# mfkiwl/HiSpMV

Hardware: AMD Instinct MI355X
Metric: SpMV GFLOP/s, SuiteSparse set (20 matrices), fp32 y=alpha*A*x+beta*y, flops=2*(nnz+rows) (higher is better)
Workload: dtype f32

## Files before the change

hispmv_amd/csrc/hispmv_kernels.hip:

```cpp
#include <hip/hip_runtime.h>

#include "hispmv_format.h"
#include "hispmv_kernels.h"
#include <algorithm>
#include <cstdlib>
#include <mutex>
#include <type_traits>
#include <vector>

#ifndef HISPMV_TTS_EXPERIMENT
#define HISPMV_TTS_EXPERIMENT 0
#endif

namespace hispmv {

#ifdef HISPMV_WG_TRACE
__device__ unsigned long long* g_wgt_buf = nullptr;
__device__ unsigned g_wgt_cap = 0;
struct WgTrace {
    unsigned long long t0;
    __device__ __forceinline__ void begin() { t0 = __builtin_amdgcn_s_memrealtime(); }
    __device__ __forceinline__ void end(int kind, int entry, long long item) {
        __syncthreads();
        if (threadIdx.x == 0 && g_wgt_buf) {
            const unsigned long long t1 = __builtin_amdgcn_s_memrealtime();
            unsigned hw, xcc;
            asm volatile("s_getreg_b32 %0, hwreg(HW_REG_HW_ID)" : "=s"(hw));
            asm volatile("s_getreg_b32 %0, hwreg(HW_REG_XCC_ID)" : "=s"(xcc));
            const unsigned long long i = __hip_atomic_fetch_add(g_wgt_buf, 1ull, __ATOMIC_RELAXED, __HIP_MEMORY_SCOPE_AGENT);
            if (i < g_wgt_cap) {
                unsigned long long* r = g_wgt_buf + 4 + 4 * i;
                r[0] = t0; r[1] = t1;
                r[2] = ((unsigned long long)xcc << 32) | hw;
                r[3] = ((unsigned long long)kind << 56) | ((unsigned long long)(entry & 0xffff) << 40) | (unsigned long long)(item & 0xffffffffffll);
            }
        }
    }
};
#define WGT_BEGIN() WgTrace wgt; wgt.begin()
#define WGT_END(kind, entry, item) wgt.end(kind, entry, item)
#else
#define WGT_BEGIN()
#define WGT_END(kind, entry, item)
#endif

__device__ __forceinline__ int f2i(float f) { return __builtin_bit_cast(int, f); }
__device__ __forceinline__ float i2f(int i) { return __builtin_bit_cast(float, i); }

struct ScanFlags { unsigned long long f[7]; };
__device__ __forceinline__ ScanFlags scan_flags(unsigned long long heads) {
    ScanFlags s;
    s.f[0] = heads;
    s.f[1] = s.f[0] | ((s.f[0] << 1) & 0xfffefffefffefffeull);
    s.f[2] = s.f[1] | ((s.f[1] << 2) & 0xfffcfffcfffcfffcull);
    s.f[3] = s.f[2] | ((s.f[2] << 4) & 0xfff0fff0fff0fff0ull);
    s.f[4] = s.f[3] | ((s.f[3] << 8) & 0xff00ff00ff00ff00ull);
    s.f[5] = s.f[4] | (((s.f[4] >> 15) & 1ull) ? 0x00000000ffff0000ull : 0ull)
                    | (((s.f[4] >> 47) & 1ull) ? 0xffff000000000000ull : 0ull);
    s.f[6] = s.f[5] | (((s.f[5] >> 31) & 1ull) ? 0xffffffff00000000ull : 0ull);
    return s;
}
template <int CTRL, int ROWMASK>
__device__ __forceinline__ void seg_scan_step(float& v, unsigned long long F) {
    const float vp = i2f(__builtin_amdgcn_update_dpp(0, f2i(v), CTRL, ROWMASK, 0xf, false));
    v = __builtin_amdgcn_inverse_ballot_w64(F) ? v : v + vp;
}
__device__ __forceinline__ void seg_scan_wave(float& v, const ScanFlags& s) {
    seg_scan_step<0x111, 0xf>(v, s.f[0]);
    seg_scan_step<0x112, 0xf>(v, s.f[1]);
    seg_scan_step<0x114, 0xf>(v, s.f[2]);
    seg_scan_step<0x118, 0xf>(v, s.f[3]);
    seg_scan_step<0x142, 0xa>(v, s.f[4]);
    seg_scan_step<0x143, 0xc>(v, s.f[5]);
}

__device__ __forceinline__ float wave_sum(float v) {
    v += i2f(__builtin_amdgcn_update_dpp(0, f2i(v), 0x111, 0xf, 0xf, false));
    v += i2f(__builtin_amdgcn_update_dpp(0, f2i(v), 0x112, 0xf, 0xf, false));
    v += i2f(__builtin_amdgcn_update_dpp(0, f2i(v), 0x114, 0xf, 0xf, false));
    v += i2f(__builtin_amdgcn_update_dpp(0, f2i(v), 0x118, 0xf, 0xf, false));
    v += i2f(__builtin_amdgcn_update_dpp(0, f2i(v), 0x142, 0xa, 0xf, false));
    v += i2f(__builtin_amdgcn_update_dpp(0, f2i(v), 0x143, 0xc, 0xf, false));
    return i2f(__builtin_amdgcn_readlane(f2i(v), 63));
}

constexpr int kTtsChunkSlots = 1024;
constexpr int kLookbackSpinMax = 1 << 22;

__device__ __forceinline__ int lanes_below(unsigned long long mask) {
    return __builtin_amdgcn_mbcnt_hi((unsigned)(mask >> 32), __builtin_amdgcn_mbcnt_lo((unsigned)mask, 0));
}

typedef __attribute__((address_space(3))) unsigned long long lds_u64;
__device__ __forceinline__ void mbox_store(lds_u64* p, unsigned long long v) {
    __hip_atomic_store(p, v, __ATOMIC_RELAXED, __HIP_MEMORY_SCOPE_WORKGROUP);
}
__device__ __forceinline__ unsigned long long mbox_load(lds_u64* p) {
    return __hip_atomic_load(p, __ATOMIC_RELAXED, __HIP_MEMORY_SCOPE_WORKGROUP);
}

__device__ __forceinline__ float lookback_chain(const LookbackArgs& lb, lds_u64* local,
                                                long long first, long long cur, int chain_len, int lane) {
    float part = 0.0f;
    for (int k = lane; k < chain_len; k += 64) {
        const long long src = cur - chain_len + k;
        unsigned long long v;
        int spins = 0;
        if (src >= first) {
            v = mbox_load(local + (src - first));
            while ((unsigned)(v >> 32) != lb.epoch && spins < kLookbackSpinMax) {
                __builtin_amdgcn_s_sleep(1);
                v = mbox_load(local + (src - first));
                ++spins;
            }
        } else {
            const unsigned long long* g = lb.gran + src;
            v = __hip_atomic_load(g, __ATOMIC_RELAXED, __HIP_MEMORY_SCOPE_AGENT);
            while ((unsigned)(v >> 32) != lb.epoch && spins < kLookbackSpinMax) {
                __builtin_amdgcn_s_sleep(2);
                v = __hip_atomic_load(g, __ATOMIC_RELAXED, __HIP_MEMORY_SCOPE_AGENT);
                ++spins;
            }
        }
        if ((unsigned)(v >> 32) != lb.epoch) *lb.err = 1;
        part += i2f((int)(unsigned)v);
    }
    return wave_sum(part);
}

#define HISPMV_GLOBAL __attribute__((address_space(1)))
__device__ __forceinline__ uint4 load_words(const uint4* p) {
    typedef unsigned int u4v __attribute__((ext_vector_type(4)));
    const u4v v = __builtin_nontemporal_load((const HISPMV_GLOBAL u4v*)p);
    return uint4{v.x, v.y, v.z, v.w};
}
__device__ __forceinline__ uint2 load_words2(const uint2* p) {
    typedef unsigned int u2v __attribute__((ext_vector_type(2)));
    const u2v v = __builtin_nontemporal_load((const HISPMV_GLOBAL u2v*)p);
    return uint2{v.x, v.y};
}
__device__ __forceinline__ int4 load_int4(const int4* p) {
    typedef int i4v __attribute__((ext_vector_type(4)));
    const i4v v = *(const HISPMV_GLOBAL i4v*)p;
    return int4{v.x, v.y, v.z, v.w};
}
__device__ __forceinline__ float4 load_float4(const float4* p) {
    typedef float f4v __attribute__((ext_vector_type(4)));
    const f4v v = *(const HISPMV_GLOBAL f4v*)p;
    return float4{v.x, v.y, v.z, v.w};
}
__device__ __forceinline__ void store_float(float* p, float v) { *(HISPMV_GLOBAL float*)p = v; }
__device__ __forceinline__ int2 load_int2(const int2* p) {
    typedef int i2v __attribute__((ext_vector_type(2)));
    const i2v v = *(const HISPMV_GLOBAL i2v*)p;
    return int2{v.x, v.y};
}

template <bool COMPACT, bool HALF = false> struct SliceRaw;
template <> struct SliceRaw<true>  { uint4 v[kSliceSteps]; uint2 m[kSliceSteps]; };
template <> struct SliceRaw<false> { uint4 v[kSliceSteps]; uint4 m[kSliceSteps]; };
template <> struct SliceRaw<true, true> { uint4 q[kSliceSteps]; };
template <bool COMPACT, bool HALF = false>
__device__ __forceinline__ void request_slice(SliceRaw<COMPACT, HALF>& s, const char* base, int lane) {
    if constexpr (HALF) {
        const uint4* pq = (const uint4*)base + lane;
#pragma unroll
        for (int j = 0; j < kSliceSteps; ++j) s.q[j] = load_words(pq + j * 64);
    } else {
    const uint4* pv = (const uint4*)base + lane;
#pragma unroll
    for (int j = 0; j < kSliceSteps; ++j) s.v[j] = load_words(pv + j * 64);
    if constexpr (COMPACT) {
        const uint2* pm = (const uint2*)(base + kSliceElems * 4) + lane;
#pragma unroll
        for (int j = 0; j < kSliceSteps; ++j) s.m[j] = load_words2(pm + j * 64);
    } else {
        const uint4* pm = (const uint4*)(base + kSliceElems * 4) + lane;
#pragma unroll
        for (int j = 0; j < kSliceSteps; ++j) s.m[j] = load_words(pm + j * 64);
    }
    }
}
template <bool COMPACT, bool HALF>
__device__ __forceinline__ void slice_values(const SliceRaw<COMPACT, HALF>& s, int j, float (&v)[kLaneElems]) {
    if constexpr (HALF) {
        v[0] = i2f((int)(s.q[j].x << 16)); v[1] = i2f((int)(s.q[j].x & 0xffff0000u));
        v[2] = i2f((int)(s.q[j].y << 16)); v[3] = i2f((int)(s.q[j].y & 0xffff0000u));
    } else {
        v[0] = i2f((int)s.v[j].x); v[1] = i2f((int)s.v[j].y); v[2] = i2f((int)s.v[j].z); v[3] = i2f((int)s.v[j].w);
    }
}
template <bool COMPACT, bool HALF = false>
__device__ __forceinline__ void decode_metas(const SliceRaw<COMPACT, HALF>& s, unsigned (&c)[kSliceSteps * kLaneElems]) {
    if constexpr (COMPACT) {
#pragma unroll
        for (int j = 0; j < kSliceSteps; ++j) {
            unsigned a, b;
            if constexpr (HALF) { a = s.q[j].z; b = s.q[j].w; } else { a = s.m[j].x; b = s.m[j].y; }
            c[4 * j + 0] = ((a & 0x8000u) << 16) | (a & 0x7fffu);
            c[4 * j + 1] = (a & 0x80000000u) | ((a >> 16) & 0x7fffu);
            c[4 * j + 2] = ((b & 0x8000u) << 16) | (b & 0x7fffu);
            c[4 * j + 3] = (b & 0x80000000u) | ((b >> 16) & 0x7fffu);
        }
    } else {
#pragma unroll
        for (int j = 0; j < kSliceSteps; ++j) { c[4 * j + 0] = s.m[j].x; c[4 * j + 1] = s.m[j].y; c[4 * j + 2] = s.m[j].z; c[4 * j + 3] = s.m[j].w; }
    }
}

__device__ __forceinline__ void scan_step(const float (&p)[kLaneElems], bool e0, bool e1, bool e2, bool e3, float& carry_step,
                                          float (&t)[kLaneElems]) {
    const float s0 = p[0];
    const float s1 = e0 ? p[1] : s0 + p[1];
    const float s2 = e1 ? p[2] : s1 + p[2];
    const float s3 = e2 ? p[3] : s2 + p[3];
    float v = e3 ? 0.0f : s3;
    const ScanFlags F = scan_flags(__builtin_amdgcn_ballot_w64(e0 | e1 | e2 | e3));
    seg_scan_wave(v, F);
    v = __builtin_amdgcn_inverse_ballot_w64(F.f[6]) ? v : v + carry_step;
    const float cin = i2f(__builtin_amdgcn_update_dpp(f2i(carry_step), f2i(v), 0x138, 0xf, 0xf, false));
    carry_step = i2f(__builtin_amdgcn_readlane(f2i(v), 63));
    t[0] = cin + s0;
    t[1] = e0 ? s1 : cin + s1;
    t[2] = (e0 | e1) ? s2 : cin + s2;
    t[3] = (e0 | e1 | e2) ? s3 : cin + s3;
}

__device__ __forceinline__ void stage_fragments(const int4* __restrict__ frags, int first, int count, const float* x, float* win,
                                                int cols, int lane, int wave, int n_waves) {
    constexpr int kU = 8;
    int4 fr = wave < count ? load_int4(frags + first + wave) : int4{0, 0, 0, 0};
    for (int f = wave; f < count; f += n_waves) {
        const int col0 = __builtin_amdgcn_readfirstlane(fr.x), n4 = __builtin_amdgcn_readfirstlane(fr.y) >> 2;
        const int off = __builtin_amdgcn_readfirstlane(fr.z);
        if (f + n_waves < count) fr = load_int4(frags + first + f + n_waves);
        const float4* src = (const float4*)(x + col0);
        float4* dst = (float4*)(win + off);
        const int inside = cols - col0 >= 4 * n4 ? n4 : (cols > col0 ? (cols - col0) >> 2 : 0);
        int i0 = 0;
        for (; inside - i0 > 128; i0 += 64 * kU) {
            float4 v[kU];
#pragma unroll
            for (int u = 0; u < kU; ++u) {
                const int i = i0 + 64 * u + lane;
                v[u] = load_float4(src + (i < inside ? i : inside - 1));
            }
#pragma unroll
            for (int u = 0; u < kU; ++u) {
                const int i = i0 + 64 * u + lane;
                if (i < inside) dst[i] = v[u];
            }
        }
        if (inside - i0 > 64) {
            const int ia = i0 + lane, ib = i0 + 64 + lane;
            const float4 va = load_float4(src + ia), vb = load_float4(src + (ib < inside ? ib : inside - 1));
            dst[ia] = va;
            if (ib < inside) dst[ib] = vb;
        } else if (inside - i0 > 0) {
            const int ia = i0 + lane;
            if (ia < inside) dst[ia] = load_float4(src + ia);
        }
        if (inside + lane < n4) {
            const int i = inside + lane, c0 = col0 + 4 * i;
            const HISPMV_GLOBAL float* xg = (const HISPMV_GLOBAL float*)x;
            const float a0 = c0 + 0 < cols ? xg[c0 + 0] : 0.f;
            const float a1 = c0 + 1 < cols ? xg[c0 + 1] : 0.f;
            const float a2 = c0 + 2 < cols ? xg[c0 + 2] : 0.f;
            dst[i] = float4{a0, a1, a2, 0.f};
        }
    }
}

struct SubBlock {
    int wave, n_waves, lds_off;
    int lane;
    static __device__ __forceinline__ SubBlock whole() { return SubBlock{(int)(threadIdx.x >> 6), (int)(blockDim.x >> 6), 0, (int)(threadIdx.x & 63)}; }
};

template <bool HAS_BETA, bool USE_LDS, bool LOOKBACK, bool COMPACT, bool STRAYS = false, bool HALF = false>
__device__ __forceinline__ void slices_group(
    const char* __restrict__ stream, const int4* __restrict__ hdr, const int4* __restrict__ groups,
    const int4* __restrict__ frags,
    const float* __restrict__ x, const float* bias, float* y,
    float* __restrict__ carry, float alpha, float beta, long long n_slices, int group_slices,
    int lds_floats, int ytile_floats, int cols, int rows, const LookbackArgs& lb, long long group, int4 g, const SubBlock sb) {
    extern __shared__ float xs_base[];
    float* const xs = xs_base + sb.lds_off;
    const __amdgpu_buffer_rsrc_t rx = __builtin_amdgcn_make_buffer_rsrc((void*)x, 0, cols * 4, 0x00020000);
    const __amdgpu_buffer_rsrc_t rb = __builtin_amdgcn_make_buffer_rsrc((void*)bias, 0, rows * 4, 0x00020000);
    const __amdgpu_buffer_rsrc_t ry = __builtin_amdgcn_make_buffer_rsrc((void*)y, 0, rows * 4, 0x00020000);
    const __amdgpu_buffer_rsrc_t rc = __builtin_amdgcn_make_buffer_rsrc((void*)carry, 0, LOOKBACK ? 0 : (int)(n_slices * 4), 0x00020000);
    constexpr unsigned kNoAccess = 0xffffffffu;
    constexpr int kE = kSliceSteps * kLaneElems;
    const int lane = sb.lane;
    const int wave = sb.wave, n_waves = sb.n_waves;
    float* const ytile = xs + (USE_LDS ? lds_floats : 0) + wave * ytile_floats;
    lds_u64* const mbox = (lds_u64*)(xs + (USE_LDS ? lds_floats : 0) + n_waves * ytile_floats);
    const long long first = group * group_slices;
    const long long last = (first + group_slices < n_slices) ? first + group_slices : n_slices;
    constexpr int slice_bytes = HALF ? kHalfSliceBytes : COMPACT ? kCompactSliceBytes : kWideSliceBytes;
    const char* const gbase = stream + (USE_LDS ? (size_t)(unsigned)__builtin_amdgcn_readfirstlane(g.z) * kSliceUnit
                                                : (size_t)first * kWideSliceBytes);

    const int n_here = (int)(last > first ? last - first : 0);
    const int rot = (LOOKBACK || n_here == 0) ? 0 : (int)((unsigned long long)group * 29ull % (unsigned)n_here);
    int k_slice = wave;
    int local = k_slice < n_here ? (k_slice + rot >= n_here ? k_slice + rot - n_here : k_slice + rot) : n_here;
    SliceRaw<COMPACT, HALF> w;
    int4 h = int4{0, 0, 0, 0};
    const bool strays = STRAYS && COMPACT && (__builtin_amdgcn_readfirstlane(g.w) & 2) != 0;
    const __amdgpu_buffer_rsrc_t rs = __builtin_amdgcn_make_buffer_rsrc((void*)(hdr + n_slices), 0, strays ? (int)(n_slices * (kStraySlots * 4)) : 0, 0x00020000);
    float* const stray_area = xs + (lds_floats - n_waves * kStraySlots) + wave * kStraySlots;
    unsigned sc_next = 0xffffffffu;
    float sx_cur = 0.0f;
    if (strays) {
        const unsigned sc0 = local < n_here ? __builtin_amdgcn_raw_buffer_load_b32(rs, (unsigned)((first + local) * kStraySlots + lane) << 2, 0, 0) : 0xffffffffu;
        const int k2 = k_slice + n_waves;
        const int l2 = k2 < n_here ? (k2 + rot >= n_here ? k2 + rot - n_here : k2 + rot) : -1;
        sc_next = l2 >= 0 ? __builtin_amdgcn_raw_buffer_load_b32(rs, (unsigned)((first + l2) * kStraySlots + lane) << 2, 0, 0) : 0xffffffffu;
        sx_cur = i2f((int)__builtin_amdgcn_raw_buffer_load_b32(rx, sc0 << 2, 0, 0));
    }
    if (local < n_here) {
        h = load_int4(hdr + first + local);
        request_slice<COMPACT, HALF>(w, gbase + (size_t)local * slice_bytes, lane);
    }

    if (LOOKBACK) {
        for (int i = threadIdx.x; i < group_slices; i += blockDim.x) mbox_store(mbox + i, 0ull);
        if (!USE_LDS) __syncthreads();
    }
    bool in_lds = false;
    if (USE_LDS) {
        in_lds = g.y > 0;
        stage_fragments(frags, g.x, g.y, x, xs, cols, lane, wave, n_waves);
        __syncthreads();
    }

    long long def_slice = -1, pend_slice = -1;
    int def_row = 0, def_len = 0, pend_row = 0, pend_len = 0;
    float def_t = 0.0f, def_b = 0.0f, pend_t = 0.0f, pend_b = 0.0f;
    float out_t0 = 0.0f, out_t1 = 0.0f, out_b0 = 0.0f, out_b1 = 0.0f, out_carry = 0.0f;
    unsigned out_d0 = kNoAccess, out_d1 = kNoAccess, out_dc = kNoAccess;

    while (local < n_here) {
        asm volatile("" :: "v"(h.x), "v"(h.y), "v"(h.z), "v"(h.w));
        int row = __builtin_amdgcn_readfirstlane(h.x);
        const int row_first = row;
        const int chain_len = __builtin_amdgcn_readfirstlane(h.y);
        const int n_rows = __builtin_amdgcn_readfirstlane(h.z);
        const bool spills = USE_LDS && __builtin_amdgcn_readfirstlane(h.w) != 0;
        unsigned c[kE];
        decode_metas<COMPACT, HALF>(w, c);
        if (!LOOKBACK) {
            asm volatile("" : "+v"(c[0]), "+v"(c[kE - 1]) :: "memory");
            __builtin_amdgcn_raw_buffer_store_b32((unsigned)f2i(HAS_BETA ? alpha * out_t0 + beta * out_b0 : alpha * out_t0), ry, out_d0, 0, 0);
            __builtin_amdgcn_raw_buffer_store_b32((unsigned)f2i(HAS_BETA ? alpha * out_t1 + beta * out_b1 : alpha * out_t1), ry, out_d1, 0, 0);
            __builtin_amdgcn_raw_buffer_store_b32((unsigned)f2i(out_carry), rc, out_dc, 0, 0);
        }
        float sx_next = 0.0f;
        if (strays) {
            stray_area[lane] = sx_cur;
            sx_next = i2f((int)__builtin_amdgcn_raw_buffer_load_b32(rx, sc_next << 2, 0, 0));
        }
        float bpre0 = 0.0f, bpre1 = 0.0f;
        if (HAS_BETA) {
            bpre0 = i2f((int)__builtin_amdgcn_raw_buffer_load_b32(rb, lane < n_rows ? (unsigned)(row_first + lane) << 2 : kNoAccess, 0, 0));
            bpre1 = i2f((int)__builtin_amdgcn_raw_buffer_load_b32(rb, lane + 64 < n_rows ? (unsigned)(row_first + lane + 64) << 2 : kNoAccess, 0, 0));
        }
        int r0[kSliceSteps];
        bool ends[kE];
        unsigned step_has_end = 0;
#pragma unroll
        for (int j = 0; j < kSliceSteps; ++j) {
            int below = 0, total = 0;
#pragma unroll
            for (int k = 0; k < kLaneElems; ++k) {
                ends[4 * j + k] = (c[4 * j + k] & kRowEndBit) != 0;
                const unsigned long long m = __builtin_amdgcn_ballot_w64(ends[4 * j + k]);
                below += lanes_below(m);
                total += __builtin_popcountll(m);
            }
            r0[j] = row + below;
            row += total;
            step_has_end |= (total != 0 ? 1u : 0u) << j;
        }

        float xv[kE];
        if (COMPACT || (USE_LDS && in_lds && !spills)) {
#pragma unroll
            for (int i = 0; i < kE; ++i) xv[i] = xs[c[i] & ~kRowEndBit];
        } else if (USE_LDS && in_lds) {
#pragma unroll
            for (int i = 0; i < kE; ++i) {
                const unsigned ci = c[i] & ~kRowEndBit;
                xv[i] = i2f((int)__builtin_amdgcn_raw_buffer_load_b32(rx, (ci & kGlobalColBit) ? ci << 2 : kNoAccess, 0, 0));
            }
#pragma unroll
            for (int i = 0; i < kE; ++i) {
                const unsigned ci = c[i] & ~kRowEndBit;
                const float l = xs[(ci & kGlobalColBit) ? 0u : ci];
                xv[i] = (ci & kGlobalColBit) ? xv[i] : l;
            }
        } else {
#pragma unroll
            for (int i = 0; i < kE; ++i) xv[i] = i2f((int)__builtin_amdgcn_raw_buffer_load_b32(rx, (c[i] & ~kRowEndBit) << 2, 0, 0));
        }
        float p[kE];
#pragma unroll
        for (int j = 0; j < kSliceSteps; ++j) {
            if constexpr (HALF) {
                float vj[kLaneElems];
                slice_values(w, j, vj);
                p[4 * j + 0] = vj[0] * xv[4 * j + 0]; p[4 * j + 1] = vj[1] * xv[4 * j + 1];
                p[4 * j + 2] = vj[2] * xv[4 * j + 2]; p[4 * j + 3] = vj[3] * xv[4 * j + 3];
            } else {
            p[4 * j + 0] = i2f((int)w.v[j].x) * xv[4 * j + 0];
            p[4 * j + 1] = i2f((int)w.v[j].y) * xv[4 * j + 1];
            p[4 * j + 2] = i2f((int)w.v[j].z) * xv[4 * j + 2];
            p[4 * j + 3] = i2f((int)w.v[j].w) * xv[4 * j + 3];
            }
        }
        if (!LOOKBACK) {
#pragma unroll
            for (int i = 0; i < kE; ++i) asm volatile("" : "+v"(p[i]));
            asm volatile("" ::: "memory");
        }
        const long long cur = first + local;
        k_slice += n_waves;
        local = k_slice < n_here ? (k_slice + rot >= n_here ? k_slice + rot - n_here : k_slice + rot) : n_here;
        if (strays) {
            const int k2 = k_slice + n_waves;
            const int l2 = k2 < n_here ? (k2 + rot >= n_here ? k2 + rot - n_here : k2 + rot) : -1;
            sx_cur = sx_next;
            sc_next = l2 >= 0 ? __builtin_amdgcn_raw_buffer_load_b32(rs, (unsigned)((first + l2) * kStraySlots + lane) << 2, 0, 0) : 0xffffffffu;
        }
        if (local < n_here) {
            h = load_int4(hdr + first + local);
            request_slice<COMPACT, HALF>(w, gbase + (size_t)local * slice_bytes, lane);
        }

        float carry_step = 0.0f;
#pragma unroll
        for (int j = 0; j < kSliceSteps; ++j) {
            if (step_has_end & (1u << j)) {
                const float pj[kLaneElems] = {p[4 * j], p[4 * j + 1], p[4 * j + 2], p[4 * j + 3]};
                float tj[kLaneElems];
                scan_step(pj, ends[4 * j], ends[4 * j + 1], ends[4 * j + 2], ends[4 * j + 3], carry_step, tj);
                int pos = r0[j] - row_first;
#pragma unroll
                for (int k = 0; k < kLaneElems; ++k) {
                    if (ends[4 * j + k]) ytile[pos] = tj[k];
                    pos += ends[4 * j + k] ? 1 : 0;
                }
            } else {
                carry_step = wave_sum(((p[4 * j] + p[4 * j + 1]) + p[4 * j + 2]) + p[4 * j + 3]) + carry_step;
            }
        }

        bool deferred = false, rolling = false;
        if (LOOKBACK) {
            if (lane == 0) {
                const unsigned long long granule = ((unsigned long long)lb.epoch << 32) | (unsigned)f2i(carry_step);
                mbox_store(mbox + (cur - first), granule);
                __hip_atomic_store(lb.gran + cur, granule, __ATOMIC_RELAXED, __HIP_MEMORY_SCOPE_AGENT);
            }
            if (pend_slice >= 0) {
                const float chain = lookback_chain(lb, mbox, first, pend_slice, pend_len, lane);
                if (lane == 0) {
                    const float tt = pend_t + chain;
                    __builtin_amdgcn_raw_buffer_store_b32((unsigned)f2i(HAS_BETA ? alpha * tt + beta * pend_b : alpha * tt), ry,
                                                          (unsigned)pend_row << 2, 0, 0);
                }
                pend_slice = -1;
            }
            deferred = chain_len > (int)(cur - first);
            rolling = chain_len > 0 && !deferred;
            if (deferred) { def_slice = cur; def_row = row_first; def_len = chain_len; }
            if (rolling) { pend_slice = cur; pend_row = row_first; pend_len = chain_len; }
        }

        const bool held = LOOKBACK && (deferred || rolling);
        if (!LOOKBACK) {
            out_t0 = lane < n_rows ? ytile[lane] : 0.0f;
            out_t1 = lane + 64 < n_rows ? ytile[lane + 64] : 0.0f;
            out_b0 = bpre0; out_b1 = bpre1;
            out_d0 = lane < n_rows ? (unsigned)(row_first + lane) << 2 : kNoAccess;
            out_d1 = lane + 64 < n_rows ? (unsigned)(row_first + lane + 64) << 2 : kNoAccess;
            out_carry = carry_step;
            out_dc = lane == 0 ? (unsigned)cur << 2 : kNoAccess;
        }
        for (int i0 = 128; !LOOKBACK && i0 < n_rows; i0 += 256) {
            float bb[4] = {0.0f, 0.0f, 0.0f, 0.0f};
            if (HAS_BETA) {
#pragma unroll
                for (int u = 0; u < 4; ++u) {
                    const int i = i0 + 64 * u + lane;
                    bb[u] = i2f((int)__builtin_amdgcn_raw_buffer_load_b32(rb, i < n_rows ? (unsigned)(row_first + i) << 2 : kNoAccess, 0, 0));
                }
            }
#pragma unroll
            for (int u = 0; u < 4; ++u) {
                const int i = i0 + 64 * u + lane;
                const float tt = i < n_rows ? ytile[i] : 0.0f;
                __builtin_amdgcn_raw_buffer_store_b32((unsigned)f2i(HAS_BETA ? alpha * tt + beta * bb[u] : alpha * tt), ry,
                                                      i < n_rows ? (unsigned)(row_first + i) << 2 : kNoAccess, 0, 0);
            }
        }
        for (int i = lane; LOOKBACK && i < n_rows; i += 64) {
            const float tt = ytile[i];
            const unsigned dst = (held && i == 0) ? kNoAccess : (unsigned)(row_first + i) << 2;
            if (HAS_BETA) {
                const float b = (i < 64) ? bpre0 : (i < 128) ? bpre1
                              : i2f((int)__builtin_amdgcn_raw_buffer_load_b32(rb, (unsigned)(row_first + i) << 2, 0, 0));
                if (LOOKBACK && deferred && i == 0) { def_t = tt; def_b = b; }
                if (LOOKBACK && rolling && i == 0) { pend_t = tt; pend_b = b; }
                __builtin_amdgcn_raw_buffer_store_b32((unsigned)f2i(alpha * tt + beta * b), ry, dst, 0, 0);
            } else {
                if (LOOKBACK && deferred && i == 0) def_t = tt;
                if (LOOKBACK && rolling && i == 0) pend_t = tt;
                __builtin_amdgcn_raw_buffer_store_b32((unsigned)f2i(alpha * tt), ry, dst, 0, 0);
            }
        }
    }
    if (!LOOKBACK) {
        __builtin_amdgcn_raw_buffer_store_b32((unsigned)f2i(HAS_BETA ? alpha * out_t0 + beta * out_b0 : alpha * out_t0), ry, out_d0, 0, 0);
        __builtin_amdgcn_raw_buffer_store_b32((unsigned)f2i(HAS_BETA ? alpha * out_t1 + beta * out_b1 : alpha * out_t1), ry, out_d1, 0, 0);
        __builtin_amdgcn_raw_buffer_store_b32((unsigned)f2i(out_carry), rc, out_dc, 0, 0);
    }
    if (LOOKBACK && pend_slice >= 0) {
        const float chain = lookback_chain(lb, mbox, first, pend_slice, pend_len, lane);
        if (lane == 0) {
            const float tt = pend_t + chain;
            __builtin_amdgcn_raw_buffer_store_b32((unsigned)f2i(HAS_BETA ? alpha * tt + beta * pend_b : alpha * tt), ry,
                                                  (unsigned)pend_row << 2, 0, 0);
        }
    }
    if (LOOKBACK && def_slice >= 0) {
        const float chain = lookback_chain(lb, mbox, first, def_slice, def_len, lane);
        if (lane == 0) {
            const float tt = def_t + chain;
            __builtin_amdgcn_raw_buffer_store_b32((unsigned)f2i(HAS_BETA ? alpha * tt + beta * def_b : alpha * tt), ry,
                                                  (unsigned)def_row << 2, 0, 0);
        }
    }
}

template <bool HAS_BETA, bool USE_LDS, bool LOOKBACK, bool STRAYS = false, int HALF = 0>
__device__ __forceinline__ void slices_body(
    const char* __restrict__ stream, const int4* __restrict__ hdr, const int4* __restrict__ groups,
    const int4* __restrict__ frags, const float* __restrict__ x, const float* bias, float* y,
    float* __restrict__ carry, float alpha, float beta, long long n_slices, int group_slices,
    int lds_floats, int ytile_floats, int cols, int rows, const LookbackArgs& lb, long long group, const SubBlock sb) {
    __shared__ long long s_group;
    if (LOOKBACK) {
        if (lb.use_ticket) {
            if (threadIdx.x == 0)
                s_group = (long long)(__hip_atomic_fetch_add(lb.ticket, 1ull, __ATOMIC_RELAXED, __HIP_MEMORY_SCOPE_AGENT) - lb.ticket_base);
            __syncthreads();
            group = s_group;
        }
    }
    if constexpr (USE_LDS) {
        const int4 g = group * group_slices < n_slices ? load_int4(groups + group) : int4{0, 0, 0, 0};
        if constexpr (HALF != 0) {
            if ((__builtin_amdgcn_readfirstlane(g.w) & kGroupHalf) != 0) {
                slices_group<HAS_BETA, true, LOOKBACK, true, STRAYS, true>(stream, hdr, groups, frags, x, bias, y, carry, alpha, beta, n_slices, group_slices,
                                                                           lds_floats, ytile_floats, cols, rows, lb, group, g, sb);
                return;
            }
        }
        if constexpr (HALF == 2) {
            slices_group<HAS_BETA, true, LOOKBACK, false>(stream, hdr, groups, frags, x, bias, y, carry, alpha, beta, n_slices, group_slices,
                                                          lds_floats, ytile_floats, cols, rows, lb, group, g, sb);
            return;
        }
        if (__builtin_amdgcn_readfirstlane(g.w) != 0)
            slices_group<HAS_BETA, true, LOOKBACK, true, STRAYS>(stream, hdr, groups, frags, x, bias, y, carry, alpha, beta, n_slices, group_slices,
                                                         lds_floats, ytile_floats, cols, rows, lb, group, g, sb);
        else
            slices_group<HAS_BETA, true, LOOKBACK, false>(stream, hdr, groups, frags, x, bias, y, carry, alpha, beta, n_slices, group_slices,
                                                          lds_floats, ytile_floats, cols, rows, lb, group, g, sb);
    } else {
        slices_group<HAS_BETA, false, LOOKBACK, false>(stream, hdr, groups, frags, x, bias, y, carry, alpha, beta, n_slices, group_slices,
                                                       lds_floats, ytile_floats, cols, rows, lb, group, int4{0, 0, 0, 0}, sb);
    }
}
template <bool HAS_BETA, bool USE_LDS, bool LOOKBACK, bool STRAYS = false, int HALF = 0>
__device__ __forceinline__ void slices_body(
    const char* __restrict__ stream, const int4* __restrict__ hdr, const int4* __restrict__ groups,
    const int4* __restrict__ frags, const float* __restrict__ x, const float* bias, float* y,
    float* __restrict__ carry, float alpha, float beta, long long n_slices, int group_slices,
    int lds_floats, int ytile_floats, int cols, int rows, const LookbackArgs& lb, long long group) {
    slices_body<HAS_BETA, USE_LDS, LOOKBACK, STRAYS, HALF>(stream, hdr, groups, frags, x, bias, y, carry, alpha, beta, n_slices, group_slices,
                                                     lds_floats, ytile_floats, cols, rows, lb, group, SubBlock::whole());
}

template <bool HAS_BETA, bool USE_LDS, bool LOOKBACK, bool STRAYS = false>
__global__ __launch_bounds__(1024) void spmv_slices_kernel(
    const char* __restrict__ words, const int4* __restrict__ hdr, const int4* __restrict__ groups,
    const int4* __restrict__ frags, const float* __restrict__ x, const float* bias, float* y,
    float* __restrict__ carry, float alpha, float beta, long long n_slices, int group_slices,
    int lds_floats, int ytile_floats, int cols, int rows, LookbackArgs lb) {
    slices_body<HAS_BETA, USE_LDS, LOOKBACK, STRAYS>(words, hdr, groups, frags, x, bias, y, carry, alpha, beta, n_slices, group_slices,
                                             lds_floats, ytile_floats, cols, rows, lb, (long long)blockIdx.x);
}

template <bool HAS_BETA, bool LOOKBACK, bool STRAYS>
__global__ __launch_bounds__(1024) void spmv_slices_half_kernel(
    const char* __restrict__ words, const int4* __restrict__ hdr, const int4* __restrict__ groups,
    const int4* __restrict__ frags, const float* __restrict__ x, const float* bias, float* y,
    float* __restrict__ carry, float alpha, float beta, long long n_slices, int group_slices,
    int lds_floats, int ytile_floats, int cols, int rows, LookbackArgs lb) {
    slices_body<HAS_BETA, true, LOOKBACK, STRAYS, 2>(words, hdr, groups, frags, x, bias, y, carry, alpha, beta, n_slices, group_slices,
                                                        lds_floats, ytile_floats, cols, rows, lb, (long long)blockIdx.x);
}

template <bool STRAYS>
__global__ __launch_bounds__(1024) void spmv_slices_multi_kernel(const MultiEntry* __restrict__ table, MultiPrefix prefix, float alpha) {
    int k = 0;
#pragma unroll 1
    while (k + 1 < prefix.n && (long long)blockIdx.x >= prefix.begin[k + 1]) ++k;
    long long group = (long long)blockIdx.x - prefix.begin[k];
    int e = prefix.first[k];
    const int tiles = prefix.tiles[k];
    if (tiles > 1) {
        const int per = 8 / tiles, res = (int)(group & 7);
        e += res / per;
        group = (group >> 3) * per + (res % per);
    }
    const MultiEntry t = table[e];
    if (group * t.group_slices >= t.n_slices) return;
    WGT_BEGIN();
    const LookbackArgs lb{};
    if (t.beta != 0.0f)
        slices_body<true, true, false, STRAYS>((const char*)t.words, t.hdr, t.groups, t.frags, t.x, t.bias, t.y, t.carry, alpha, t.beta,
                                       t.n_slices, t.group_slices, t.lds_floats, t.ytile_floats, t.cols, t.rows, lb, group);
    else
        slices_body<false, true, false, STRAYS>((const char*)t.words, t.hdr, t.groups, t.frags, t.x, t.y, t.y, t.carry, alpha, 0.0f,
                                        t.n_slices, t.group_slices, t.lds_floats, t.ytile_floats, t.cols, t.rows, lb, group);
    WGT_END(blockDim.x == 1024 ? 1 : 2, e, group);
}
template <bool STRAYS>
__global__ __launch_bounds__(1024) void spmv_slices_multi_half_kernel(const MultiEntry* __restrict__ table, MultiPrefix prefix, float alpha) {
    int k = 0;
#pragma unroll 1
    while (k + 1 < prefix.n && (long long)blockIdx.x >= prefix.begin[k + 1]) ++k;
    long long group = (long long)blockIdx.x - prefix.begin[k];
    int e = prefix.first[k];
    const int tiles = prefix.tiles[k];
    if (tiles > 1) {
        const int per = 8 / tiles, res = (int)(group & 7);
        e += res / per;
        group = (group >> 3) * per + (res % per);
    }
    const MultiEntry t = table[e];
    if (group * t.group_slices >= t.n_slices) return;
    WGT_BEGIN();
    const LookbackArgs lb{};
    if (t.beta != 0.0f)
        slices_body<true, true, false, STRAYS, 1>((const char*)t.words, t.hdr, t.groups, t.frags, t.x, t.bias, t.y, t.carry, alpha, t.beta,
                                       t.n_slices, t.group_slices, t.lds_floats, t.ytile_floats, t.cols, t.rows, lb, group);
    else
        slices_body<false, true, false, STRAYS, 1>((const char*)t.words, t.hdr, t.groups, t.frags, t.x, t.y, t.y, t.carry, alpha, 0.0f,
                                        t.n_slices, t.group_slices, t.lds_floats, t.ytile_floats, t.cols, t.rows, lb, group);
    WGT_END(blockDim.x == 1024 ? 1 : 2, e, group);
}
__global__ __launch_bounds__(256) void spmv_fixup_multi_kernel(const MultiFixEntry* __restrict__ table, MultiPrefix prefix, float alpha) {
    int e = 0;
#pragma unroll 1
    while (e + 1 < prefix.n && (long long)blockIdx.x >= prefix.begin[e + 1]) ++e;
    const MultiFixEntry t = table[e];
    const int i = (int)(blockIdx.x - prefix.begin[e]) * blockDim.x + threadIdx.x;
    if (i >= t.n) return;
    const int4 f = t.fix[i];
    float s = 0.0f;
    for (int k = 0; k < f.z; ++k) s += t.carry[f.y + k];
    t.y[f.x] += alpha * s;
}

__global__ __launch_bounds__(256) void spmv_merge_parts_kernel(float* __restrict__ y, const float* __restrict__ parts, int n_parts,
                                                               long long part_stride, int rows, long long y_stride, long long vec_stride) {
    const int i = blockIdx.x * blockDim.x + threadIdx.x;
    if (i >= rows) return;
    y += blockIdx.y * y_stride;
    parts += blockIdx.y * vec_stride;
    float s = y[i];
    for (int t = 0; t < n_parts; ++t) s += parts[(size_t)t * part_stride + i];
    y[i] = s;
}
__global__ __launch_bounds__(256) void spmv_merge_multi_kernel(const MultiMergeEntry* __restrict__ table, MultiPrefix prefix) {
    int e = 0;
#pragma unroll 1
    while (e + 1 < prefix.n && (long long)blockIdx.x >= prefix.begin[e + 1]) ++e;
    const MultiMergeEntry t = table[e];
    const int i = (int)(blockIdx.x - prefix.begin[e]) * blockDim.x + threadIdx.x;
    if (i >= t.rows) return;
    float s = t.y[i];
    for (int k = 0; k < t.n_parts; ++k) s += t.parts[(size_t)k * t.part_stride + i];
    t.y[i] = s;
}

__global__ __launch_bounds__(256) void spmv_tail_multi_kernel(const MultiFixEntry* __restrict__ fix_table, MultiPrefix fix_prefix,
                                                              const TailMergeEntry* __restrict__ merge_table, MultiPrefix merge_prefix, float alpha) {
    const long long n_fix_blocks = fix_prefix.begin[fix_prefix.n];
    if ((long long)blockIdx.x < n_fix_blocks) {
        int e = 0;
#pragma unroll 1
        while (e + 1 < fix_prefix.n && (long long)blockIdx.x >= fix_prefix.begin[e + 1]) ++e;
        const MultiFixEntry t = fix_table[e];
        const int i = (int)(blockIdx.x - fix_prefix.begin[e]) * blockDim.x + threadIdx.x;
        if (i >= t.n) return;
        const int4 f = t.fix[i];
        float s = 0.0f;
        for (int k = 0; k < f.z; ++k) s += t.carry[f.y + k];
        t.y[f.x] += alpha * s;
        return;
    }
    const long long b = (long long)blockIdx.x - n_fix_blocks;
    int e = 0;
#pragma unroll 1
    while (e + 1 < merge_prefix.n && b >= merge_prefix.begin[e + 1]) ++e;
    const TailMergeEntry& t = merge_table[e];
    const int rows = t.rows, n_parts = t.n_parts;
    const int i = (int)(b - merge_prefix.begin[e]) * blockDim.x + threadIdx.x;
    if (i >= rows) return;
    const int32_t* fr = t.fix_of_row;
    float s = t.y[i];
    for (int q = 0; q <= n_parts; ++q) {
        float v = q == 0 ? s : t.parts[(size_t)(q - 1) * t.part_stride + i];
        const int fi = fr ? fr[(size_t)q * rows + i] : -1;
        if (fi >= 0) {
            const int4 f = t.fix[q][fi];
            const float* cy = t.carry[q];
            float c = 0.0f;
            for (int k = 0; k < f.z; ++k) c += cy[f.y + k];
            v += alpha * c;
        }
        s = q == 0 ? v : s + v;
    }
    t.y[i] = s;
}

template <bool HAS_BETA, bool USE_LDS, int NV, bool COMPACT, bool HALF = false>
__device__ __forceinline__ void batched_group(
    const char* __restrict__ stream, const int4* __restrict__ hdr,
    const int4* __restrict__ frags,
    const float* __restrict__ x, const float* bias, float* y,
    float* __restrict__ carry, float alpha, float beta, long long n_slices, int group_slices,
    int lds_floats, int ytile_floats, int cols, int rows, int bias_stride, int4 g) {
    extern __shared__ float xs[];
    const __amdgpu_buffer_rsrc_t rx = __builtin_amdgcn_make_buffer_rsrc((void*)x, 0, cols * NV * 4, 0x00020000);
    const __amdgpu_buffer_rsrc_t rb = __builtin_amdgcn_make_buffer_rsrc((void*)bias, 0, (bias_stride ? rows * NV : rows) * 4, 0x00020000);
    const __amdgpu_buffer_rsrc_t ry = __builtin_amdgcn_make_buffer_rsrc((void*)y, 0, rows * NV * 4, 0x00020000);
    constexpr unsigned kNoAccess = 0xffffffffu;
    constexpr int kE = kSliceSteps * kLaneElems;
    const int lane = threadIdx.x & 63;
    const int wave = threadIdx.x >> 6, n_waves = blockDim.x >> 6;
    float* const ytile = xs + (USE_LDS ? NV * lds_floats : 0) + wave * ytile_floats;
    const long long group = blockIdx.x;
    const long long first = group * group_slices;
    const long long last = (first + group_slices < n_slices) ? first + group_slices : n_slices;
    constexpr int slice_bytes = HALF ? kHalfSliceBytes : COMPACT ? kCompactSliceBytes : kWideSliceBytes;
    const char* const gbase = stream + (USE_LDS ? (size_t)(unsigned)__builtin_amdgcn_readfirstlane(g.z) * kSliceUnit
                                                : (size_t)first * kWideSliceBytes);

    const int n_here = (int)(last > first ? last - first : 0);
    const int rot = n_here == 0 ? 0 : (int)((unsigned long long)group * 29ull % (unsigned)n_here);
    int k_slice = wave;
    auto local_at = [&](int k) { return k < n_here ? (k + rot >= n_here ? k + rot - n_here : k + rot) : n_here; };
    long long slice = first + local_at(k_slice);
    const bool strays = COMPACT && (__builtin_amdgcn_readfirstlane(g.w) & 2) != 0;
    const __amdgpu_buffer_rsrc_t rs = __builtin_amdgcn_make_buffer_rsrc((void*)(hdr + n_slices), 0, strays ? (int)(n_slices * (kStraySlots * 4)) : 0, 0x00020000);
    unsigned sc = 0xffffffffu;
    SliceRaw<COMPACT, HALF> w;
    int4 h = int4{0, 0, 0, 0};
    if (slice < last) {
        if (strays) sc = __builtin_amdgcn_raw_buffer_load_b32(rs, (unsigned)(slice * kStraySlots + lane) << 2, 0, 0);
        h = load_int4(hdr + slice);
        request_slice<COMPACT, HALF>(w, gbase + (size_t)(slice - first) * slice_bytes, lane);
    }
    bool in_lds = false;
    if (USE_LDS) {
        in_lds = g.y > 0;
        for (int v = 0; v < NV; ++v) {
            const float* xv = x + (size_t)v * cols;
            stage_fragments(frags, g.x, g.y, xv, xs + v * lds_floats, cols, lane, wave, n_waves);
        }
        __syncthreads();
    }

    while (slice < last) {
        int row = __builtin_amdgcn_readfirstlane(h.x);
        const int row_first = row;
        const int n_rows = __builtin_amdgcn_readfirstlane(h.z);
        const bool spills = USE_LDS && __builtin_amdgcn_readfirstlane(h.w) != 0;
        unsigned c[kE];
        decode_metas<COMPACT, HALF>(w, c);
        float val[HALF ? 1 : kE];
        unsigned hv[HALF ? 2 * kSliceSteps : 1];
#pragma unroll
        for (int j = 0; j < kSliceSteps; ++j) {
            if constexpr (HALF) {
                hv[2 * j] = w.q[j].x; hv[2 * j + 1] = w.q[j].y;
            } else {
            val[4 * j + 0] = i2f((int)w.v[j].x); val[4 * j + 1] = i2f((int)w.v[j].y);
            val[4 * j + 2] = i2f((int)w.v[j].z); val[4 * j + 3] = i2f((int)w.v[j].w);
            }
        }
        int r0[kSliceSteps];
        bool ends[kE];
#pragma unroll
        for (int j = 0; j < kSliceSteps; ++j) {
            int below = 0, total = 0;
#pragma unroll
            for (int k = 0; k < kLaneElems; ++k) {
                ends[4 * j + k] = (c[4 * j + k] & kRowEndBit) != 0;
                const unsigned long long m = __builtin_amdgcn_ballot_w64(ends[4 * j + k]);
                below += lanes_below(m);
                total += __builtin_popcountll(m);
            }
            r0[j] = row + below;
            row += total;
        }
        const long long cur = slice;
        if (strays) {
            float sx[NV];
#pragma unroll
            for (int v = 0; v < NV; ++v)
                sx[v] = i2f((int)__builtin_amdgcn_raw_buffer_load_b32(rx, sc == 0xffffffffu ? kNoAccess : (sc + (unsigned)v * (unsigned)cols) << 2, 0, 0));
#pragma unroll
            for (int v = 0; v < NV; ++v) (xs + v * lds_floats + (lds_floats - n_waves * kStraySlots) + wave * kStraySlots)[lane] = sx[v];
        }

#pragma unroll
        for (int v = 0; v < NV; ++v) {
            const unsigned xoff = (unsigned)v * (unsigned)cols, yoff = (unsigned)v * (unsigned)rows;
            const unsigned boff = (unsigned)v * (unsigned)bias_stride;
            float bpre0 = 0.0f, bpre1 = 0.0f;
            if (HAS_BETA) {
                bpre0 = i2f((int)__builtin_amdgcn_raw_buffer_load_b32(rb, lane < n_rows ? (boff + row_first + lane) << 2 : kNoAccess, 0, 0));
                bpre1 = i2f((int)__builtin_amdgcn_raw_buffer_load_b32(rb, lane + 64 < n_rows ? (boff + row_first + lane + 64) << 2 : kNoAccess, 0, 0));
            }
            float xg[kE];
            const float* xw = xs + v * lds_floats;
            if (USE_LDS && in_lds && !spills) {
#pragma unroll
                for (int i = 0; i < kE; ++i) xg[i] = xw[c[i] & ~kRowEndBit];
            } else if (USE_LDS && in_lds) {
#pragma unroll
                for (int i = 0; i < kE; ++i) {
                    const unsigned ci = c[i] & ~kRowEndBit;
                    xg[i] = i2f((int)__builtin_amdgcn_raw_buffer_load_b32(rx, (ci & kGlobalColBit) ? ((ci & ~kGlobalColBit) + xoff) << 2 : kNoAccess, 0, 0));
                }
#pragma unroll
                for (int i = 0; i < kE; ++i) {
                    const unsigned ci = c[i] & ~kRowEndBit;
                    const float l = xw[(ci & kGlobalColBit) ? 0u : ci];
                    xg[i] = (ci & kGlobalColBit) ? xg[i] : l;
                }
            } else {
#pragma unroll
                for (int i = 0; i < kE; ++i) xg[i] = i2f((int)__builtin_amdgcn_raw_buffer_load_b32(rx, ((c[i] & ~kRowEndBit) + xoff) << 2, 0, 0));
            }
            if (v == NV - 1) {
                k_slice += n_waves;
                slice = first + local_at(k_slice);
                if (slice < last) {
                    if (strays) sc = __builtin_amdgcn_raw_buffer_load_b32(rs, (unsigned)(slice * kStraySlots + lane) << 2, 0, 0);
                    h = load_int4(hdr + slice);
                    request_slice<COMPACT, HALF>(w, gbase + (size_t)(slice - first) * slice_bytes, lane);
                }
            }
            float t[kE];
            float carry_step = 0.0f;
#pragma unroll
            for (int j = 0; j < kSliceSteps; ++j) {
                float pj[kLaneElems];
                if constexpr (HALF) {
                    pj[0] = i2f((int)(hv[2 * j] << 16)) * xg[4 * j]; pj[1] = i2f((int)(hv[2 * j] & 0xffff0000u)) * xg[4 * j + 1];
                    pj[2] = i2f((int)(hv[2 * j + 1] << 16)) * xg[4 * j + 2]; pj[3] = i2f((int)(hv[2 * j + 1] & 0xffff0000u)) * xg[4 * j + 3];
// ... 1097 lines not shown
```

Before: 1295.

## Keep two compact slices in flight per wave with hand-counted vmcnt waits

Adds a two-deep software pipeline for compact fp32 LDS groups. Each wave issues raw inline-asm global loads for the next slice (header, values, metas; non-temporal) while it computes the current one, and defers its y, carry and bias stores and loads into the next iteration. A manual s_waitcnt vmcnt(9) is used so only the older slice has to land. It also rotates slice order per group. The aim is to hide memory latency in this bandwidth-bound SpMV, at the cost of more VGPRs (possibly lower occupancy) and fragile manual waitcnt bookkeeping.

```diff
diff --git a/hispmv_amd/csrc/hispmv_kernels.hip b/hispmv_amd/csrc/hispmv_kernels.hip
--- a/hispmv_amd/csrc/hispmv_kernels.hip
+++ b/hispmv_amd/csrc/hispmv_kernels.hip
@@ -181,6 +181,51 @@
     }
     }
 }
+constexpr int kDeepLoads = 1 + 2 * kSliceSteps;
+typedef unsigned int hispmv_u4v __attribute__((ext_vector_type(4)));
+typedef int hispmv_i4v __attribute__((ext_vector_type(4)));
+struct SliceRegs { hispmv_u4v v[kSliceSteps]; unsigned long long m[kSliceSteps]; hispmv_i4v h; };
+__device__ __forceinline__ void request_slice_uncounted(SliceRegs& s, const int4* hp, const char* base, int lane) {
+    static_assert(kSliceSteps == 4 && kSliceElems * 4 == 4096, "the offsets below are those of the compact slice");
+    const char* const pv = base + lane * 16;
+    const char* const pm = base + kSliceElems * 4 + lane * 8;
+    asm volatile("global_load_dwordx4 %[h], %[hp], off\n\t"
+                 "global_load_dwordx4 %[v0], %[pv], off nt\n\t"
+                 "global_load_dwordx4 %[v1], %[pv], off offset:1024 nt\n\t"
+                 "global_load_dwordx4 %[v2], %[pv], off offset:2048 nt\n\t"
+                 "global_load_dwordx4 %[v3], %[pv], off offset:3072 nt\n\t"
+                 "global_load_dwordx2 %[m0], %[pm], off nt\n\t"
+                 "global_load_dwordx2 %[m1], %[pm], off offset:512 nt\n\t"
+                 "global_load_dwordx2 %[m2], %[pm], off offset:1024 nt\n\t"
+                 "global_load_dwordx2 %[m3], %[pm], off offset:1536 nt"
+                 : [h] "=&v"(s.h), [v0] "=&v"(s.v[0]), [v1] "=&v"(s.v[1]), [v2] "=&v"(s.v[2]), [v3] "=&v"(s.v[3]),
+                   [m0] "=&v"(s.m[0]), [m1] "=&v"(s.m[1]), [m2] "=&v"(s.m[2]), [m3] "=&v"(s.m[3])
+                 : [hp] "v"(hp), [pv] "v"(pv), [pm] "v"(pm)
+                 : "memory");
+}
+__device__ __forceinline__ void request_bias_uncounted(float& b0, float& b1, __amdgpu_buffer_rsrc_t rb, unsigned off0, unsigned off1) {
+    asm volatile("s_nop 4\n\t"
+                 "buffer_load_dword %[b0], %[o0], %[rb], 0 offen\n\t"
+                 "buffer_load_dword %[b1], %[o1], %[rb], 0 offen"
+                 : [b0] "+v"(b0), [b1] "+v"(b1)
+                 : [o0] "v"(off0), [o1] "v"(off1), [rb] "s"(rb)
+                 : "memory");
+}
+__device__ __forceinline__ void await_slice_uncounted(SliceRegs& s, float& b0, float& b1, int younger) {
+    static_assert(kDeepLoads == 9, "the count in the string");
+    asm volatile("s_cmp_eq_u32 %[y], 0\n\t"
+                 "s_cbranch_scc1 .Lhispmv_drain_%=\n\t"
+                 "s_waitcnt vmcnt(9)\n\t"
+                 "s_branch .Lhispmv_landed_%=\n"
+                 ".Lhispmv_drain_%=:\n\t"
+                 "s_waitcnt vmcnt(0)\n"
+                 ".Lhispmv_landed_%=:"
+                 : "+v"(s.h), "+v"(s.v[0]), "+v"(s.v[1]), "+v"(s.v[2]), "+v"(s.v[3]), "+v"(s.m[0]), "+v"(s.m[1]), "+v"(s.m[2]), "+v"(s.m[3]),
+                   "+v"(b0), "+v"(b1)
+                 : [y] "s"(younger)
+                 : "scc");
+}
+
 template <bool COMPACT, bool HALF>
 __device__ __forceinline__ void slice_values(const SliceRaw<COMPACT, HALF>& s, int j, float (&v)[kLaneElems]) {
     if constexpr (HALF) {
@@ -190,13 +235,15 @@
         v[0] = i2f((int)s.v[j].x); v[1] = i2f((int)s.v[j].y); v[2] = i2f((int)s.v[j].z); v[3] = i2f((int)s.v[j].w);
     }
 }
-template <bool COMPACT, bool HALF = false>
-__device__ __forceinline__ void decode_metas(const SliceRaw<COMPACT, HALF>& s, unsigned (&c)[kSliceSteps * kLaneElems]) {
+template <bool COMPACT, bool HALF = false, class Raw>
+__device__ __forceinline__ void decode_metas(const Raw& s, unsigned (&c)[kSliceSteps * kLaneElems]) {
     if constexpr (COMPACT) {
 #pragma unroll
         for (int j = 0; j < kSliceSteps; ++j) {
             unsigned a, b;
-            if constexpr (HALF) { a = s.q[j].z; b = s.q[j].w; } else { a = s.m[j].x; b = s.m[j].y; }
+            if constexpr (HALF) { a = s.q[j].z; b = s.q[j].w; }
+            else if constexpr (sizeof(s.m[j]) == sizeof(uint2) && !__is_same(Raw, SliceRaw<true>)) { a = (unsigned)s.m[j]; b = (unsigned)(s.m[j] >> 32); }
+            else { a = s.m[j].x; b = s.m[j].y; }
             c[4 * j + 0] = ((a & 0x8000u) << 16) | (a & 0x7fffu);
             c[4 * j + 1] = (a & 0x80000000u) | ((a >> 16) & 0x7fffu);
             c[4 * j + 2] = ((b & 0x8000u) << 16) | (b & 0x7fffu);
@@ -277,13 +324,157 @@
     static __device__ __forceinline__ SubBlock whole() { return SubBlock{(int)(threadIdx.x >> 6), (int)(blockDim.x >> 6), 0, (int)(threadIdx.x & 63)}; }
 };
 
-template <bool HAS_BETA, bool USE_LDS, bool LOOKBACK, bool COMPACT, bool STRAYS = false, bool HALF = false>
+template <bool HAS_BETA>
+__device__ __forceinline__ void slices_group_two_deep(
+    const char* __restrict__ stream, const int4* __restrict__ hdr, const int4* __restrict__ frags,
+    const float* __restrict__ x, const float* bias, float* y,
+    float* __restrict__ carry, float alpha, float beta, long long n_slices, int group_slices,
+    int lds_floats, int ytile_floats, int cols, int rows, long long group, int4 g, const SubBlock sb) {
+    extern __shared__ float xs_base[];
+    float* const xs = xs_base + sb.lds_off;
+    const __amdgpu_buffer_rsrc_t rb = __builtin_amdgcn_make_buffer_rsrc((void*)bias, 0, rows * 4, 0x00020000);
+    const __amdgpu_buffer_rsrc_t ry = __builtin_amdgcn_make_buffer_rsrc((void*)y, 0, rows * 4, 0x00020000);
+    const __amdgpu_buffer_rsrc_t rc = __builtin_amdgcn_make_buffer_rsrc((void*)carry, 0, (int)(n_slices * 4), 0x00020000);
+    constexpr unsigned kNoAccess = 0xffffffffu;
+    constexpr int kE = kSliceSteps * kLaneElems;
+    const int lane = sb.lane;
+    const int wave = sb.wave, n_waves = sb.n_waves;
+    float* const ytile = xs + lds_floats + wave * ytile_floats;
+    const long long first = group * group_slices;
+    const long long last = (first + group_slices < n_slices) ? first + group_slices : n_slices;
+    const char* const gbase = stream + (size_t)(unsigned)__builtin_amdgcn_readfirstlane(g.z) * kSliceUnit;
+    const int n_here = (int)(last > first ? last - first : 0);
+    const int rot = n_here == 0 ? 0 : (int)((unsigned long long)group * 29ull % (unsigned)n_here);
+    auto local_at = [&](int k) { return k < n_here ? (k + rot >= n_here ? k + rot - n_here : k + rot) : n_here; };
+    int k_slice = wave;
+    int local_a = local_at(k_slice), local_b = local_at(k_slice + n_waves);
+    SliceRegs wa, wb;
+    wa.h = wb.h = hispmv_i4v{0, 0, 0, 0};
+    if (local_a < n_here) request_slice_uncounted(wa, hdr + first + local_a, gbase + (size_t)local_a * kCompactSliceBytes, lane);
+    if (local_b < n_here) request_slice_uncounted(wb, hdr + first + local_b, gbase + (size_t)local_b * kCompactSliceBytes, lane);
+    stage_fragments(frags, g.x, g.y, x, xs, cols, lane, wave, n_waves);
+    __syncthreads();
+
+    float out_t0 = 0.0f, out_t1 = 0.0f, out_b0 = 0.0f, out_b1 = 0.0f, out_carry = 0.0f;
+    unsigned out_d0 = kNoAccess, out_d1 = kNoAccess, out_dc = kNoAccess;
+
+    auto one_slice = [&](SliceRegs& w, int& local, int younger) __attribute__((always_inline)) {
+        await_slice_uncounted(w, out_b0, out_b1, younger);
+        int row = __builtin_amdgcn_readfirstlane(w.h.x);
+        const int row_first = row;
+        const int n_rows = __builtin_amdgcn_readfirstlane(w.h.z);
+        unsigned c[kE];
+        decode_metas<true, false>(w, c);
+#pragma unroll
+        for (int i = 1; i < kE - 1; ++i) asm volatile("" : "+v"(c[i]));
+        asm volatile("" : "+v"(c[0]), "+v"(c[kE - 1]) :: "memory");
+        __builtin_amdgcn_raw_buffer_store_b32((unsigned)f2i(HAS_BETA ? alpha * out_t0 + beta * out_b0 : alpha * out_t0), ry, out_d0, 0, 0);
+        __builtin_amdgcn_raw_buffer_store_b32((unsigned)f2i(HAS_BETA ? alpha * out_t1 + beta * out_b1 : alpha * out_t1), ry, out_d1, 0, 0);
+        __builtin_amdgcn_raw_buffer_store_b32((unsigned)f2i(out_carry), rc, out_dc, 0, 0);
+        if (HAS_BETA) request_bias_uncounted(out_b0, out_b1, rb, lane < n_rows ? (unsigned)(row_first + lane) << 2 : kNoAccess,
+                                             lane + 64 < n_rows ? (unsigned)(row_first + lane + 64) << 2 : kNoAccess);
+        int r0[kSliceSteps];
+        bool ends[kE];
+        unsigned step_has_end = 0;
+#pragma unroll
+        for (int j = 0; j < kSliceSteps; ++j) {
+            int below = 0, total = 0;
+#pragma unroll
+            for (int k = 0; k < kLaneElems; ++k) {
+                ends[4 * j + k] = (c[4 * j + k] & kRowEndBit) != 0;
+                const unsigned long long m = __builtin_amdgcn_ballot_w64(ends[4 * j + k]);
+                below += lanes_below(m);
+                total += __builtin_popcountll(m);
+            }
+            r0[j] = row + below;
+            row += total;
+            step_has_end |= (total != 0 ? 1u : 0u) << j;
+        }
+        float xv[kE];
+#pragma unroll
+        for (int i = 0; i < kE; ++i) xv[i] = xs[c[i] & ~kRowEndBit];
+        float p[kE];
+#pragma unroll
+        for (int j = 0; j < kSliceSteps; ++j) {
+            p[4 * j + 0] = i2f((int)w.v[j].x) * xv[4 * j + 0];
+            p[4 * j + 1] = i2f((int)w.v[j].y) * xv[4 * j + 1];
+            p[4 * j + 2] = i2f((int)w.v[j].z) * xv[4 * j + 2];
+            p[4 * j + 3] = i2f((int)w.v[j].w) * xv[4 * j + 3];
+        }
+#pragma unroll
+        for (int i = 0; i < kE; ++i) asm volatile("" : "+v"(p[i]));
+        asm volatile("" ::: "memory");
+        const long long cur = first + local;
+        k_slice += n_waves;
+        local = local_at(k_slice + n_waves);
+        SliceRegs next;
+        if (local < n_here) request_slice_uncounted(next, hdr + first + local, gbase + (size_t)local * kCompactSliceBytes, lane);
+        w = next;
+
+        float carry_step = 0.0f;
+#pragma unroll
+        for (int j = 0; j < kSliceSteps; ++j) {
+            if (step_has_end & (1u << j)) {
+                const float pj[kLaneElems] = {p[4 * j], p[4 * j + 1], p[4 * j + 2], p[4 * j + 3]};
+                float tj[kLaneElems];
+                scan_step(pj, ends[4 * j], ends[4 * j + 1], ends[4 * j + 2], ends[4 * j + 3], carry_step, tj);
+                int pos = r0[j] - row_first;
+#pragma unroll
+                for (int k = 0; k < kLaneElems; ++k) {
+                    if (ends[4 * j + k]) ytile[pos] = tj[k];
+                    pos += ends[4 * j + k] ? 1 : 0;
+                }
+            } else {
+                carry_step = wave_sum(((p[4 * j] + p[4 * j + 1]) + p[4 * j + 2]) + p[4 * j + 3]) + carry_step;
+            }
+        }
+        out_t0 = lane < n_rows ? ytile[lane] : 0.0f;
+        out_t1 = lane + 64 < n_rows ? ytile[lane + 64] : 0.0f;
+        out_d0 = lane < n_rows ? (unsigned)(row_first + lane) << 2 : kNoAccess;
+        out_d1 = lane + 64 < n_rows ? (unsigned)(row_first + lane + 64) << 2 : kNoAccess;
+        out_carry = carry_step;
+        out_dc = lane == 0 ? (unsigned)cur << 2 : kNoAccess;
+        for (int i0 = 128; i0 < n_rows; i0 += 256) {
+            float bb[4] = {0.0f, 0.0f, 0.0f, 0.0f};
+            if (HAS_BETA) {
+#pragma unroll
+                for (int u = 0; u < 4; ++u) {
+                    const int i = i0 + 64 * u + lane;
+                    bb[u] = i2f((int)__builtin_amdgcn_raw_buffer_load_b32(rb, i < n_rows ? (unsigned)(row_first + i) << 2 : kNoAccess, 0, 0));
+                }
+            }
+#pragma unroll
+            for (int u = 0; u < 4; ++u) {
+                const int i = i0 + 64 * u + lane;
+                const float tt = i < n_rows ? ytile[i] : 0.0f;
+                __builtin_amdgcn_raw_buffer_store_b32((unsigned)f2i(HAS_BETA ? alpha * tt + beta * bb[u] : alpha * tt), ry,
+                                                      i < n_rows ? (unsigned)(row_first + i) << 2 : kNoAccess, 0, 0);
+            }
+        }
+    };
+    while (local_a < n_here) {
+        one_slice(wa, local_a, __builtin_amdgcn_readfirstlane(local_b < n_here ? 1 : 0));
+        if (!(local_b < n_here)) break;
+        one_slice(wb, local_b, __builtin_amdgcn_readfirstlane(local_a < n_here ? 1 : 0));
+    }
+    if (HAS_BETA) asm volatile("s_waitcnt vmcnt(0)" : "+v"(out_b0), "+v"(out_b1));
+    __builtin_amdgcn_raw_buffer_store_b32((unsigned)f2i(HAS_BETA ? alpha * out_t0 + beta * out_b0 : alpha * out_t0), ry, out_d0, 0, 0);
+    __builtin_amdgcn_raw_buffer_store_b32((unsigned)f2i(HAS_BETA ? alpha * out_t1 + beta * out_b1 : alpha * out_t1), ry, out_d1, 0, 0);
+    __builtin_amdgcn_raw_buffer_store_b32((unsigned)f2i(out_carry), rc, out_dc, 0, 0);
+}
+
+template <bool HAS_BETA, bool USE_LDS, bool LOOKBACK, bool COMPACT, bool STRAYS = false, bool HALF = false, int DEPTH = 1>
 __device__ __forceinline__ void slices_group(
     const char* __restrict__ stream, const int4* __restrict__ hdr, const int4* __restrict__ groups,
     const int4* __restrict__ frags,
     const float* __restrict__ x, const float* bias, float* y,
     float* __restrict__ carry, float alpha, float beta, long long n_slices, int group_slices,
     int lds_floats, int ytile_floats, int cols, int rows, const LookbackArgs& lb, long long group, int4 g, const SubBlock sb) {
+    if constexpr (DEPTH == 2) {
+        static_assert(USE_LDS && COMPACT && !HALF && !LOOKBACK && !STRAYS, "two slices in flight: compact fp32 groups only");
+        slices_group_two_deep<HAS_BETA>(stream, hdr, frags, x, bias, y, carry, alpha, beta, n_slices, group_slices, lds_floats, ytile_floats, cols, rows, group, g, sb);
+        return;
+    }
     extern __shared__ float xs_base[];
     float* const xs = xs_base + sb.lds_off;
     const __amdgpu_buffer_rsrc_t rx = __builtin_amdgcn_make_buffer_rsrc((void*)x, 0, cols * 4, 0x00020000);
@@ -575,7 +766,7 @@
             return;
         }
         if (__builtin_amdgcn_readfirstlane(g.w) != 0)
-            slices_group<HAS_BETA, true, LOOKBACK, true, STRAYS>(stream, hdr, groups, frags, x, bias, y, carry, alpha, beta, n_slices, group_slices,
+            slices_group<HAS_BETA, true, LOOKBACK, true, STRAYS, false, (LOOKBACK || STRAYS) ? 1 : 2>(stream, hdr, groups, frags, x, bias, y, carry, alpha, beta, n_slices, group_slices,
                                                          lds_floats, ytile_floats, cols, rows, lb, group, g, sb);
         else
             slices_group<HAS_BETA, true, LOOKBACK, false>(stream, hdr, groups, frags, x, bias, y, carry, alpha, beta, n_slices, group_slices,
```

After: 1272. 0.982x the previous value.
